# edogariu/artist-style-transfer

Hardware: NVIDIA B200
Metric: train_images_per_sec_256 (higher is better)
Workload: dtype bf16

## Files before the change

artist_style_transfer_b200/csrc/conv_px.cu:

```cuda
#include "px_common.cuh"

namespace ast {

constexpr int PX_THREADS = 320;
constexpr int PX_MAX_STAGES = 8;
constexpr int PX_PRODUCERS = 4;

struct PxParams {
  int mi, mj, tw, th, tiles_i, tiles_j, n_img;
  int ntaps, kchunks, kc;
  int si, so, oy0, ox0;
  int cout, flags;
  int w_rows_per_img;
  int stages, w_bytes, a_bytes, stage_bytes, rowb;
  int pairs_per_img;
  unsigned idesc, layout_type, sbo;
  long long total_pairs;
  short dy[AST_MAX_TAPS];
  short dx[AST_MAX_TAPS];
};

template <int KIND>
__global__ void __launch_bounds__(PX_THREADS, 1)
conv_px_kernel(const __grid_constant__ CUtensorMap tm_in, const __grid_constant__ CUtensorMap tm_w, const PxParams p,
               const float* __restrict__ bias, const Img32 add, const Img32 mask, const Img32 out,
               double* __restrict__ stats) {
  extern __shared__ unsigned char smem_raw[];
  __shared__ __align__(8) unsigned long long full_bar[PX_MAX_STAGES], empty_bar[PX_MAX_STAGES], tfull_bar[2], tempty_bar[2];
  __shared__ unsigned tmem_slot;
  unsigned char* smem = (unsigned char*)(((uintptr_t)smem_raw + 1023) & ~(uintptr_t)1023);
  const int warp = threadIdx.x >> 5, lane = threadIdx.x & 31;
  const int ksteps = p.ntaps * p.kchunks;

  if (threadIdx.x == 0) {
    asm volatile("prefetch.tensormap [%0];" ::"l"(&tm_in) : "memory");
    asm volatile("prefetch.tensormap [%0];" ::"l"(&tm_w) : "memory");
    for (int s = 0; s < p.stages; ++s) { mbar_init(&full_bar[s], 1); mbar_init(&empty_bar[s], 1); }
    for (int a = 0; a < 2; ++a) { mbar_init(&tfull_bar[a], 1); mbar_init(&tempty_bar[a], 256); }
    asm volatile("fence.mbarrier_init.release.cluster;" ::: "memory");
    asm volatile("fence.proxy.async.shared::cta;" ::: "memory");
  }
  if (warp == 1) {
    asm volatile("tcgen05.alloc.cta_group::1.sync.aligned.shared::cta.b32 [%0], %1;" ::"r"(smem_u32(&tmem_slot)), "r"(512u) : "memory");
    asm volatile("tcgen05.relinquish_alloc_permit.cta_group::1.sync.aligned;" ::: "memory");
  }
  tc_fence_before();
  __syncthreads();
  tc_fence_after();
  const unsigned tmem_base = tmem_slot;

  if (warp == 0) {
    const int nprod = p.stages < PX_PRODUCERS ? p.stages : PX_PRODUCERS;
    if (lane < nprod) {
      int s = 0, turn = 0; unsigned ph = 0;
      for (long long pair = blockIdx.x; pair < p.total_pairs; pair += gridDim.x) {
        const int img = (int)(pair / p.pairs_per_img);
        const int sp0 = 2 * (int)(pair % p.pairs_per_img);
        const int ti0 = sp0 / p.tiles_j, tj0 = sp0 - ti0 * p.tiles_j;
        const int ti1 = (sp0 + 1) / p.tiles_j, tj1 = (sp0 + 1) - ti1 * p.tiles_j;
        const int x0 = p.si * tj0 * p.tw, y0 = p.si * ti0 * p.th, x1 = p.si * tj1 * p.tw, y1 = p.si * ti1 * p.th;
        const int wrow0 = img * p.w_rows_per_img;
        for (int t = 0; t < p.ntaps; ++t) {
          for (int kc = 0; kc < p.kchunks; ++kc) {
            if (turn == lane) {
              mbar_wait(&empty_bar[s], ph ^ 1);
              unsigned char* sw = smem + (size_t)s * p.stage_bytes;
              mbar_expect_tx(&full_bar[s], (unsigned)p.stage_bytes);
              tma_load_2d(sw, &tm_w, &full_bar[s], kc * p.kc, wrow0 + t * p.cout);
              tma_load_4d(sw + p.w_bytes, &tm_in, &full_bar[s], kc * p.kc, x0 + p.dx[t], y0 + p.dy[t], img);
              tma_load_4d(sw + p.w_bytes + p.a_bytes, &tm_in, &full_bar[s], kc * p.kc, x1 + p.dx[t], y1 + p.dy[t], img);
            }
            if (++turn == nprod) turn = 0;
            if (++s == p.stages) { s = 0; ph ^= 1; }
          }
        }
      }
    }
  } else if (warp == 1) {
    int s = 0; unsigned ph = 0; int as = 0; unsigned aph = 0;
    const int kmma = p.rowb / 32;
    const unsigned desc_hi = (p.sbo >> 4) | (1u << 14) | (p.layout_type << 29);
    for (long long pair = blockIdx.x; pair < p.total_pairs; pair += gridDim.x) {
      mbar_wait(&tempty_bar[as], aph ^ 1);
      tc_fence_after();
      const unsigned d_tmem = tmem_base + (unsigned)(as * 256);
      for (int ks = 0; ks < ksteps; ++ks) {
        mbar_wait(&full_bar[s], ph);
        tc_fence_after();
        if (lane == 0) {
          const unsigned w_addr = smem_u32(smem + (size_t)s * p.stage_bytes);
          const unsigned a_lo = ((w_addr & 0x3FFFFu) >> 4) | (1u << 16);
          const unsigned b_lo = (((w_addr + p.w_bytes) & 0x3FFFFu) >> 4) | (1u << 16);
          tc_mma<KIND>(d_tmem, pack_desc64(a_lo, desc_hi), pack_desc64(b_lo, desc_hi), p.idesc, ks > 0 ? 1u : 0u);
          tc_mma<KIND>(d_tmem, pack_desc64(a_lo + 2, desc_hi), pack_desc64(b_lo + 2, desc_hi), p.idesc, 1u);
          if (kmma == 4) {
            tc_mma<KIND>(d_tmem, pack_desc64(a_lo + 4, desc_hi), pack_desc64(b_lo + 4, desc_hi), p.idesc, 1u);
            tc_mma<KIND>(d_tmem, pack_desc64(a_lo + 6, desc_hi), pack_desc64(b_lo + 6, desc_hi), p.idesc, 1u);
          }
          tc_commit(&empty_bar[s]);
          if (ks == ksteps - 1) tc_commit(&tfull_bar[as]);
        }
        __syncwarp();
        if (++s == p.stages) { s = 0; ph ^= 1; }
      }
      if (++as == 2) { as = 0; aph ^= 1; }
    }
  } else {
    const int q = warp & 3;
    const int half = (warp - 2) >> 2;
    const int ch = q * 32 + lane;
    const bool ch_ok = ch < p.cout;
    const float b = (bias && ch_ok) ? bias[ch] : 0.f;
    int as = 0; unsigned aph = 0;
    double s1 = 0.0, s2 = 0.0;
    int s_img = -1;
    for (long long pair = blockIdx.x; pair < p.total_pairs; pair += gridDim.x) {
      const int img = (int)(pair / p.pairs_per_img);
      if (stats && img != s_img) {
        if (s_img >= 0 && ch_ok) { double* srow = stats + ((long long)s_img * p.cout + ch) * 2; atomicAdd(srow, s1); atomicAdd(srow + 1, s2); }
        s1 = s2 = 0.0; s_img = img;
      }
      const int sp = 2 * (int)(pair % p.pairs_per_img) + half;
      const int ti = sp / p.tiles_j, tj = sp - ti * p.tiles_j;
      mbar_wait(&tfull_bar[as], aph);
      tc_fence_after();
      const unsigned taddr0 = tmem_base + ((unsigned)(q * 32) << 16) + (unsigned)(as * 256 + half * 128);
      if (q * 32 < p.cout) {
        const bool fast = (p.tw & 31) == 0;
        for (int c0 = 0; c0 < 128; c0 += 32) {
          float v[32];
          tc_ld32(taddr0 + c0, v);
          if (fast) {
            const int ty = c0 / p.tw, tx0 = c0 - ty * p.tw;
            const int i = ti * p.th + ty, j0 = tj * p.tw + tx0;
            const int oy = p.oy0 + p.so * i, ox = p.ox0 + p.so * j0;
            int nvalid = 0;
            if (i < p.mi && oy < out.h) {
              const int jlim = min(p.mj, (out.w - p.ox0 + p.so - 1) / p.so);
              nvalid = max(0, min(32, jlim - j0));
            }
            PxOff off;
            off.out = img * out.sn + oy * out.sh + ox * out.sw;
            off.add = add.ptr ? img * add.sn + oy * add.sh + ox * add.sw : 0;
            off.mask = mask.ptr ? img * mask.sn + oy * mask.sh + ox * mask.sw : 0;
            PxStep st;
            st.out_r = st.add_r = st.mask_r = 0;
            st.out_c = p.so * out.sw; st.add_c = p.so * add.sw; st.mask_c = p.so * mask.sw;
            if (nvalid > 0) px_chunk<32>(v, off, st, 1, nvalid, ch, lane, b, p.flags, add, mask, out, stats != nullptr, s1, s2);
          } else {
            const int row = c0 + lane;
            const int ty = row / p.tw, tx = row - ty * p.tw;
            const int i = ti * p.th + ty, j = tj * p.tw + tx;
            const int oy = p.oy0 + p.so * i, ox = p.ox0 + p.so * j;
            const bool valid = i < p.mi && j < p.mj && oy < out.h && ox < out.w;
            PxOff off;
            off.out = valid ? img * out.sn + oy * out.sh + ox * out.sw : -1;
            off.add = add.ptr ? img * add.sn + oy * add.sh + ox * add.sw : 0;
            off.mask = mask.ptr ? img * mask.sn + oy * mask.sh + ox * mask.sw : 0;
            PxStep st = {0, 0, 0, 0, 0, 0};
            px_chunk<0>(v, off, st, 0, 0, ch, lane, b, p.flags, add, mask, out, stats != nullptr, s1, s2);
          }
        }
      }
      tc_fence_before();
      mbar_arrive(&tempty_bar[as]);
      if (++as == 2) { as = 0; aph ^= 1; }
    }
    if (stats && s_img >= 0 && ch_ok) { double* srow = stats + ((long long)s_img * p.cout + ch) * 2; atomicAdd(srow, s1); atomicAdd(srow + 1, s2); }
  }

  tc_fence_before();
  __syncthreads();
  if (warp == 1) {
    tc_fence_after();
    asm volatile("tcgen05.dealloc.cta_group::1.sync.aligned.b32 %0, %1;" ::"r"(tmem_base), "r"(512u) : "memory");
  }
}

int conv_gather_px(const ast_image* in, const void* weights, const float* bias, const ast_image* add,
                   const ast_image* mask, const ast_image* out, const ast_gather_geom* g, int cpad, bool thin,
                   cudaStream_t stream) {
  if (thin || g->pooled || (cpad != 64 && cpad != 128) || out->c != cpad) return 0;
  if (!img32_ok(out) || !img32_ok(add) || !img32_ok(mask)) return 0;
  if (in->dtype == AST_F16) return 0;
  const int esz = in->dtype == AST_F32 ? 4 : 2;
  EncodeTiledFn encode = get_encode();
  if (!encode) return 0;

  PxParams p;
  memset(&p, 0, sizeof(p));
  p.mi = g->mi; p.mj = g->mj; p.si = g->si; p.so = g->so; p.oy0 = g->oy0; p.ox0 = g->ox0;
  p.ntaps = g->ntaps; p.flags = g->flags; p.cout = cpad; p.n_img = in->n;
  for (int t = 0; t < g->ntaps; ++t) { p.dy[t] = g->dy[t]; p.dx[t] = g->dx[t]; }
  pick_tile(p.mi, p.mj, 128, &p.tw, &p.th);
  p.tiles_i = (p.mi + p.th - 1) / p.th;
  p.tiles_j = (p.mj + p.tw - 1) / p.tw;
  p.rowb = (in->c * esz) % 128 == 0 ? 128 : 64;
  p.kc = p.rowb / esz;
  p.kchunks = in->c / p.kc;
  if (p.ntaps * p.kchunks * (p.rowb / 32) < 16) return 0;
  p.w_rows_per_img = 0;
  if (g->w_img_stride) {
    if (g->w_img_stride != (int64_t)g->ntaps * cpad * in->c) return 0;
    p.w_rows_per_img = g->ntaps * cpad;
  }
  p.w_bytes = 128 * p.rowb;
  p.a_bytes = 128 * p.rowb;
  p.stage_bytes = p.w_bytes + 2 * p.a_bytes;
  p.stages = (200 * 1024) / p.stage_bytes;
  if (p.stages > PX_MAX_STAGES) p.stages = PX_MAX_STAGES;
  p.layout_type = p.rowb == 128 ? 2u : 4u;
  p.sbo = 8u * p.rowb;
  const unsigned fmt = tc_operand_fmt(in->dtype);
  p.idesc = (1u << 4) | (fmt << 7) | (fmt << 10) | ((256u >> 3) << 17) | ((128u >> 4) << 24);
  p.pairs_per_img = (p.tiles_i * p.tiles_j + 1) / 2;
  p.total_pairs = (long long)p.n_img * p.pairs_per_img;

  alignas(64) CUtensorMap tm_in, tm_w;
  const CUtensorMapDataType dt = tc_tmap_dtype(in->dtype);
  const CUtensorMapSwizzle sw = p.rowb == 128 ? CU_TENSOR_MAP_SWIZZLE_128B : CU_TENSOR_MAP_SWIZZLE_64B;
  {
    cuuint64_t dims[4] = {(cuuint64_t)in->c, (cuuint64_t)in->w, (cuuint64_t)in->h, (cuuint64_t)in->n};
    cuuint64_t strides[3] = {(cuuint64_t)in->sw * esz, (cuuint64_t)in->sh * esz, (cuuint64_t)in->sn * esz};
    cuuint32_t box[4] = {(cuuint32_t)p.kc, (cuuint32_t)(p.tw * p.si), (cuuint32_t)(p.th * p.si), 1};
    cuuint32_t estr[4] = {1, (cuuint32_t)p.si, (cuuint32_t)p.si, 1};
    if (int r = cached_tensor_map(encode, &tm_in, dt, 4, in->ptr, dims, strides, box, estr, sw, CU_TENSOR_MAP_L2_PROMOTION_L2_128B)) return r;
  }
  {
    const long long rows = (long long)g->ntaps * cpad * (g->w_img_stride ? in->n : 1);
    cuuint64_t dims[2] = {(cuuint64_t)in->c, (cuuint64_t)rows};
    cuuint64_t strides[1] = {(cuuint64_t)in->c * esz};
    cuuint32_t box[2] = {(cuuint32_t)p.kc, 128};
    cuuint32_t estr[2] = {1, 1};
    if (int r = cached_tensor_map(encode, &tm_w, dt, 2, const_cast<void*>(weights), dims, strides, box, estr, sw, CU_TENSOR_MAP_L2_PROMOTION_L2_256B)) return r;
  }
  const size_t smem = (size_t)p.stages * p.stage_bytes + 1024;
  const int grid = (int)(p.total_pairs < num_sms() ? p.total_pairs : num_sms());
  cudaError_t e;
  if (in->dtype != AST_F32) {
    e = set_max_smem(conv_px_kernel<0>, smem);
    if (e == cudaSuccess) launch_k(conv_px_kernel<0>, grid, PX_THREADS, smem, stream, tm_in, tm_w, p, bias, to_img32(add), to_img32(mask), to_img32(out), g->stats);
  } else {
    e = set_max_smem(conv_px_kernel<1>, smem);
    if (e == cudaSuccess) launch_k(conv_px_kernel<1>, grid, PX_THREADS, smem, stream, tm_in, tm_w, p, bias, to_img32(add), to_img32(mask), to_img32(out), g->stats);
  }
  if (e != cudaSuccess) { set_error("conv_px: cudaFuncSetAttribute failed: %s", cudaGetErrorString(e)); return (int)e; }
  count_launch();
  count_work(FAM_CONV_PX, conv_flops(in, out, g), conv_bytes(in, out, g, add, mask));
  AST_CUDA_LAUNCH_CHECK();
  return 1;
}

}
```

Baseline: 3465.

## Use M=64 MMA for 64-channel convs, merge pair tiles into one TMA box

For 64-output-channel convolutions the kernel now issues MMAs with M equal to the padded channel count. It loads only cpad weight rows and reads TMEM with the 16x32bx2 layout, so it no longer wastes half the tensor-core work and weight bandwidth on padding. Producer lanes in one warp become separate producer warps (two extra warps, 384 threads). Vertically adjacent tile pairs are fetched with one doubled TMA box, the tile shape is chosen to minimise padding, and the epilogue takes a uniform full-chunk fast path. The per-channel cout guard is dropped and the warp/thread layout changes, which adds register pressure and correctness risk for the TMEM lane mapping.

```diff
diff --git a/artist_style_transfer_b200/csrc/conv_px.cu b/artist_style_transfer_b200/csrc/conv_px.cu
--- a/artist_style_transfer_b200/csrc/conv_px.cu
+++ b/artist_style_transfer_b200/csrc/conv_px.cu
@@ -2,9 +2,25 @@
 
 namespace ast {
 
-constexpr int PX_THREADS = 320;
+constexpr int PX_THREADS = 384;
 constexpr int PX_MAX_STAGES = 8;
-constexpr int PX_PRODUCERS = 4;
+constexpr int PX_PRODUCERS = 3;
+
+__device__ __forceinline__ void tc_ld16x2_32(unsigned taddr, float* v) {
+  unsigned r[32];
+  asm volatile(
+      "tcgen05.ld.sync.aligned.16x32bx2.x32.b32 "
+      "{%0, %1, %2, %3, %4, %5, %6, %7, %8, %9, %10, %11, %12, %13, %14, %15, "
+      "%16, %17, %18, %19, %20, %21, %22, %23, %24, %25, %26, %27, %28, %29, %30, %31}, [%32], 32;"
+      : "=r"(r[0]), "=r"(r[1]), "=r"(r[2]), "=r"(r[3]), "=r"(r[4]), "=r"(r[5]), "=r"(r[6]), "=r"(r[7]), "=r"(r[8]),
+        "=r"(r[9]), "=r"(r[10]), "=r"(r[11]), "=r"(r[12]), "=r"(r[13]), "=r"(r[14]), "=r"(r[15]), "=r"(r[16]),
+        "=r"(r[17]), "=r"(r[18]), "=r"(r[19]), "=r"(r[20]), "=r"(r[21]), "=r"(r[22]), "=r"(r[23]), "=r"(r[24]),
+        "=r"(r[25]), "=r"(r[26]), "=r"(r[27]), "=r"(r[28]), "=r"(r[29]), "=r"(r[30]), "=r"(r[31])
+      : "r"(taddr));
+  asm volatile("tcgen05.wait::ld.sync.aligned;" ::: "memory");
+#pragma unroll
+  for (int i = 0; i < 32; ++i) v[i] = __uint_as_float(r[i]);
+}
 
 struct PxParams {
   int mi, mj, tw, th, tiles_i, tiles_j, n_img;
@@ -13,6 +29,7 @@
   int cout, flags;
   int w_rows_per_img;
   int stages, w_bytes, a_bytes, stage_bytes, rowb;
+  int pair_box;
   int pairs_per_img;
   unsigned idesc, layout_type, sbo;
   long long total_pairs;
@@ -20,7 +37,7 @@
   short dx[AST_MAX_TAPS];
 };
 
-template <int KIND>
+template <int KIND, bool M64>
 __global__ void __launch_bounds__(PX_THREADS, 1)
 conv_px_kernel(const __grid_constant__ CUtensorMap tm_in, const __grid_constant__ CUtensorMap tm_w, const PxParams p,
                const float* __restrict__ bias, const Img32 add, const Img32 mask, const Img32 out,
@@ -49,9 +66,10 @@
   tc_fence_after();
   const unsigned tmem_base = tmem_slot;
 
-  if (warp == 0) {
+  if (warp == 0 || warp >= 10) {
     const int nprod = p.stages < PX_PRODUCERS ? p.stages : PX_PRODUCERS;
-    if (lane < nprod) {
+    const int pid = warp == 0 ? 0 : warp - 9;
+    if (lane == 0 && pid < nprod) {
       int s = 0, turn = 0; unsigned ph = 0;
       for (long long pair = blockIdx.x; pair < p.total_pairs; pair += gridDim.x) {
         const int img = (int)(pair / p.pairs_per_img);
@@ -62,13 +80,14 @@
         const int wrow0 = img * p.w_rows_per_img;
         for (int t = 0; t < p.ntaps; ++t) {
           for (int kc = 0; kc < p.kchunks; ++kc) {
-            if (turn == lane) {
+            if (turn == pid) {
               mbar_wait(&empty_bar[s], ph ^ 1);
               unsigned char* sw = smem + (size_t)s * p.stage_bytes;
               mbar_expect_tx(&full_bar[s], (unsigned)p.stage_bytes);
               tma_load_2d(sw, &tm_w, &full_bar[s], kc * p.kc, wrow0 + t * p.cout);
-              tma_load_4d(sw + p.w_bytes, &tm_in, &full_bar[s], kc * p.kc, x0 + p.dx[t], y0 + p.dy[t], img);
-              tma_load_4d(sw + p.w_bytes + p.a_bytes, &tm_in, &full_bar[s], kc * p.kc, x1 + p.dx[t], y1 + p.dy[t], img);
+              sw += p.w_bytes;
+              tma_load_4d(sw, &tm_in, &full_bar[s], kc * p.kc, x0 + p.dx[t], y0 + p.dy[t], img);
+              if (!p.pair_box) tma_load_4d(sw + p.a_bytes, &tm_in, &full_bar[s], kc * p.kc, x1 + p.dx[t], y1 + p.dy[t], img);
             }
             if (++turn == nprod) turn = 0;
             if (++s == p.stages) { s = 0; ph ^= 1; }
@@ -89,8 +108,9 @@
         tc_fence_after();
         if (lane == 0) {
           const unsigned w_addr = smem_u32(smem + (size_t)s * p.stage_bytes);
+          const unsigned x_addr = w_addr + p.w_bytes;
           const unsigned a_lo = ((w_addr & 0x3FFFFu) >> 4) | (1u << 16);
-          const unsigned b_lo = (((w_addr + p.w_bytes) & 0x3FFFFu) >> 4) | (1u << 16);
+          const unsigned b_lo = ((x_addr & 0x3FFFFu) >> 4) | (1u << 16);
           tc_mma<KIND>(d_tmem, pack_desc64(a_lo, desc_hi), pack_desc64(b_lo, desc_hi), p.idesc, ks > 0 ? 1u : 0u);
           tc_mma<KIND>(d_tmem, pack_desc64(a_lo + 2, desc_hi), pack_desc64(b_lo + 2, desc_hi), p.idesc, 1u);
           if (kmma == 4) {
@@ -108,16 +128,21 @@
   } else {
     const int q = warp & 3;
     const int half = (warp - 2) >> 2;
-    const int ch = q * 32 + lane;
-    const bool ch_ok = ch < p.cout;
-    const float b = (bias && ch_ok) ? bias[ch] : 0.f;
+    const int ch = M64 ? q * 16 + (lane & 15) : q * 32 + lane;
+    const int col_lane = M64 ? (lane >> 4) * 32 : 0;
+    constexpr int chunk = M64 ? 64 : 32;
+    const float b = bias ? bias[ch] : 0.f;
     int as = 0; unsigned aph = 0;
     double s1 = 0.0, s2 = 0.0;
     int s_img = -1;
+    auto flush = [&]() {
+      if (M64) { s1 += __shfl_xor_sync(0xffffffffu, s1, 16); s2 += __shfl_xor_sync(0xffffffffu, s2, 16); }
+      if (!M64 || lane < 16) { double* srow = stats + ((long long)s_img * p.cout + ch) * 2; atomicAdd(srow, s1); atomicAdd(srow + 1, s2); }
+    };
     for (long long pair = blockIdx.x; pair < p.total_pairs; pair += gridDim.x) {
       const int img = (int)(pair / p.pairs_per_img);
       if (stats && img != s_img) {
-        if (s_img >= 0 && ch_ok) { double* srow = stats + ((long long)s_img * p.cout + ch) * 2; atomicAdd(srow, s1); atomicAdd(srow + 1, s2); }
+        if (s_img >= 0) flush();
         s1 = s2 = 0.0; s_img = img;
       }
       const int sp = 2 * (int)(pair % p.pairs_per_img) + half;
@@ -125,48 +150,34 @@
       mbar_wait(&tfull_bar[as], aph);
       tc_fence_after();
       const unsigned taddr0 = tmem_base + ((unsigned)(q * 32) << 16) + (unsigned)(as * 256 + half * 128);
-      if (q * 32 < p.cout) {
-        const bool fast = (p.tw & 31) == 0;
-        for (int c0 = 0; c0 < 128; c0 += 32) {
-          float v[32];
-          tc_ld32(taddr0 + c0, v);
-          if (fast) {
-            const int ty = c0 / p.tw, tx0 = c0 - ty * p.tw;
-            const int i = ti * p.th + ty, j0 = tj * p.tw + tx0;
-            const int oy = p.oy0 + p.so * i, ox = p.ox0 + p.so * j0;
-            int nvalid = 0;
-            if (i < p.mi && oy < out.h) {
-              const int jlim = min(p.mj, (out.w - p.ox0 + p.so - 1) / p.so);
-              nvalid = max(0, min(32, jlim - j0));
-            }
-            PxOff off;
-            off.out = img * out.sn + oy * out.sh + ox * out.sw;
-            off.add = add.ptr ? img * add.sn + oy * add.sh + ox * add.sw : 0;
-            off.mask = mask.ptr ? img * mask.sn + oy * mask.sh + ox * mask.sw : 0;
-            PxStep st;
-            st.out_r = st.add_r = st.mask_r = 0;
-            st.out_c = p.so * out.sw; st.add_c = p.so * add.sw; st.mask_c = p.so * mask.sw;
-            if (nvalid > 0) px_chunk<32>(v, off, st, 1, nvalid, ch, lane, b, p.flags, add, mask, out, stats != nullptr, s1, s2);
-          } else {
-            const int row = c0 + lane;
-            const int ty = row / p.tw, tx = row - ty * p.tw;
-            const int i = ti * p.th + ty, j = tj * p.tw + tx;
-            const int oy = p.oy0 + p.so * i, ox = p.ox0 + p.so * j;
-            const bool valid = i < p.mi && j < p.mj && oy < out.h && ox < out.w;
-            PxOff off;
-            off.out = valid ? img * out.sn + oy * out.sh + ox * out.sw : -1;
-            off.add = add.ptr ? img * add.sn + oy * add.sh + ox * add.sw : 0;
-            off.mask = mask.ptr ? img * mask.sn + oy * mask.sh + ox * mask.sw : 0;
-            PxStep st = {0, 0, 0, 0, 0, 0};
-            px_chunk<0>(v, off, st, 0, 0, ch, lane, b, p.flags, add, mask, out, stats != nullptr, s1, s2);
-          }
-        }
+      for (int c0 = 0; c0 < 128; c0 += chunk) {
+        float v[32];
+        if (M64) tc_ld16x2_32(taddr0 + c0, v);
+        else tc_ld32(taddr0 + c0, v);
+        const int ilim = min(p.mi, (out.h - p.oy0 + p.so - 1) / p.so);
+        const int jlim = min(p.mj, (out.w - p.ox0 + p.so - 1) / p.so);
+        const int col = c0 + col_lane;
+        const int ty = col / p.tw, tx0 = col - ty * p.tw;
+        const int i = ti * p.th + ty, j0 = tj * p.tw + tx0;
+        const int nvalid = i < ilim ? max(0, min(32, jlim - j0)) : 0;
+        const int oy = p.oy0 + p.so * i, ox = p.ox0 + p.so * j0;
+        PxOff off;
+        off.out = img * out.sn + oy * out.sh + ox * out.sw;
+        off.add = add.ptr ? img * add.sn + oy * add.sh + ox * add.sw : 0;
+        off.mask = mask.ptr ? img * mask.sn + oy * mask.sh + ox * mask.sw : 0;
+        PxStep st;
+        st.out_r = p.so * out.sh; st.add_r = p.so * add.sh; st.mask_r = p.so * mask.sh;
+        st.out_c = p.so * out.sw; st.add_c = p.so * add.sw; st.mask_c = p.so * mask.sw;
+        if (__all_sync(0xffffffffu, nvalid == 32))
+          px_chunk<32, true>(v, off, st, 1, 32, ch, lane, b, p.flags, add, mask, out, stats != nullptr, s1, s2);
+        else if (__any_sync(0xffffffffu, nvalid > 0))
+          px_chunk<32>(v, off, st, 1, nvalid, ch, lane, b, p.flags, add, mask, out, stats != nullptr, s1, s2);
       }
       tc_fence_before();
       mbar_arrive(&tempty_bar[as]);
       if (++as == 2) { as = 0; aph ^= 1; }
     }
-    if (stats && s_img >= 0 && ch_ok) { double* srow = stats + ((long long)s_img * p.cout + ch) * 2; atomicAdd(srow, s1); atomicAdd(srow + 1, s2); }
+    if (stats && s_img >= 0) flush();
   }
 
   tc_fence_before();
@@ -175,6 +186,13 @@
     tc_fence_after();
     asm volatile("tcgen05.dealloc.cta_group::1.sync.aligned.b32 %0, %1;" ::"r"(tmem_base), "r"(512u) : "memory");
   }
+}
+
+typedef void (*PxLaunch)(const CUtensorMap, const CUtensorMap, const PxParams, const float*, const Img32, const Img32,
+                         const Img32, double*);
+static PxLaunch px_kernel(bool tf32, bool m64) {
+  if (tf32) return m64 ? conv_px_kernel<1, true> : conv_px_kernel<1, false>;
+  return m64 ? conv_px_kernel<0, true> : conv_px_kernel<0, false>;
 }
 
 int conv_gather_px(const ast_image* in, const void* weights, const float* bias, const ast_image* add,
@@ -192,7 +210,14 @@
   p.mi = g->mi; p.mj = g->mj; p.si = g->si; p.so = g->so; p.oy0 = g->oy0; p.ox0 = g->ox0;
   p.ntaps = g->ntaps; p.flags = g->flags; p.cout = cpad; p.n_img = in->n;
   for (int t = 0; t < g->ntaps; ++t) { p.dy[t] = g->dy[t]; p.dx[t] = g->dx[t]; }
-  pick_tile(p.mi, p.mj, 128, &p.tw, &p.th);
+  {
+    double best = -1;
+    for (int w = 128; w >= 32; w >>= 1) {
+      const int h = 128 / w;
+      const double eff = (double)p.mi * p.mj / ((double)((p.mi + h - 1) / h * h) * ((p.mj + w - 1) / w * w));
+      if (eff > best + 1e-9) { best = eff; p.tw = w; p.th = h; }
+    }
+  }
   p.tiles_i = (p.mi + p.th - 1) / p.th;
   p.tiles_j = (p.mj + p.tw - 1) / p.tw;
   p.rowb = (in->c * esz) % 128 == 0 ? 128 : 64;
@@ -204,7 +229,7 @@
     if (g->w_img_stride != (int64_t)g->ntaps * cpad * in->c) return 0;
     p.w_rows_per_img = g->ntaps * cpad;
   }
-  p.w_bytes = 128 * p.rowb;
+  p.w_bytes = cpad * p.rowb;
   p.a_bytes = 128 * p.rowb;
   p.stage_bytes = p.w_bytes + 2 * p.a_bytes;
   p.stages = (200 * 1024) / p.stage_bytes;
@@ -212,8 +237,9 @@
   p.layout_type = p.rowb == 128 ? 2u : 4u;
   p.sbo = 8u * p.rowb;
   const unsigned fmt = tc_operand_fmt(in->dtype);
-  p.idesc = (1u << 4) | (fmt << 7) | (fmt << 10) | ((256u >> 3) << 17) | ((128u >> 4) << 24);
+  p.idesc = (1u << 4) | (fmt << 7) | (fmt << 10) | ((256u >> 3) << 17) | (((unsigned)cpad >> 4) << 24);
   p.pairs_per_img = (p.tiles_i * p.tiles_j + 1) / 2;
+  p.pair_box = p.tiles_j == 1 && 2 * p.th * p.si <= 256;
   p.total_pairs = (long long)p.n_img * p.pairs_per_img;
 
   alignas(64) CUtensorMap tm_in, tm_w;
@@ -222,7 +248,7 @@
   {
     cuuint64_t dims[4] = {(cuuint64_t)in->c, (cuuint64_t)in->w, (cuuint64_t)in->h, (cuuint64_t)in->n};
     cuuint64_t strides[3] = {(cuuint64_t)in->sw * esz, (cuuint64_t)in->sh * esz, (cuuint64_t)in->sn * esz};
-    cuuint32_t box[4] = {(cuuint32_t)p.kc, (cuuint32_t)(p.tw * p.si), (cuuint32_t)(p.th * p.si), 1};
+    cuuint32_t box[4] = {(cuuint32_t)p.kc, (cuuint32_t)(p.tw * p.si), (cuuint32_t)((p.pair_box ? 2 : 1) * p.th * p.si), 1};
     cuuint32_t estr[4] = {1, (cuuint32_t)p.si, (cuuint32_t)p.si, 1};
     if (int r = cached_tensor_map(encode, &tm_in, dt, 4, in->ptr, dims, strides, box, estr, sw, CU_TENSOR_MAP_L2_PROMOTION_L2_128B)) return r;
   }
@@ -230,20 +256,15 @@
     const long long rows = (long long)g->ntaps * cpad * (g->w_img_stride ? in->n : 1);
     cuuint64_t dims[2] = {(cuuint64_t)in->c, (cuuint64_t)rows};
     cuuint64_t strides[1] = {(cuuint64_t)in->c * esz};
-    cuuint32_t box[2] = {(cuuint32_t)p.kc, 128};
+    cuuint32_t box[2] = {(cuuint32_t)p.kc, (cuuint32_t)cpad};
     cuuint32_t estr[2] = {1, 1};
     if (int r = cached_tensor_map(encode, &tm_w, dt, 2, const_cast<void*>(weights), dims, strides, box, estr, sw, CU_TENSOR_MAP_L2_PROMOTION_L2_256B)) return r;
   }
   const size_t smem = (size_t)p.stages * p.stage_bytes + 1024;
   const int grid = (int)(p.total_pairs < num_sms() ? p.total_pairs : num_sms());
-  cudaError_t e;
-  if (in->dtype != AST_F32) {
-    e = set_max_smem(conv_px_kernel<0>, smem);
-    if (e == cudaSuccess) launch_k(conv_px_kernel<0>, grid, PX_THREADS, smem, stream, tm_in, tm_w, p, bias, to_img32(add), to_img32(mask), to_img32(out), g->stats);
-  } else {
-    e = set_max_smem(conv_px_kernel<1>, smem);
-    if (e == cudaSuccess) launch_k(conv_px_kernel<1>, grid, PX_THREADS, smem, stream, tm_in, tm_w, p, bias, to_img32(add), to_img32(mask), to_img32(out), g->stats);
-  }
+  const PxLaunch launch = px_kernel(in->dtype == AST_F32, cpad == 64);
+  cudaError_t e = set_max_smem(launch, smem);
+  if (e == cudaSuccess) launch_k(launch, grid, PX_THREADS, smem, stream, tm_in, tm_w, p, bias, to_img32(add), to_img32(mask), to_img32(out), g->stats);
   if (e != cudaSuccess) { set_error("conv_px: cudaFuncSetAttribute failed: %s", cudaGetErrorString(e)); return (int)e; }
   count_launch();
   count_work(FAM_CONV_PX, conv_flops(in, out, g), conv_bytes(in, out, g, add, mask));
diff --git a/scratch/conv_px_launches.py b/scratch/conv_px_launches.py
--- /dev/null
+++ b/scratch/conv_px_launches.py
@@ -0,0 +1,98 @@
+import argparse
+import json
+import os
+import subprocess
+import sys
+
+ROOT = os.path.dirname(os.path.dirname(os.path.abspath(__file__)))
+sys.path.insert(0, ROOT)
+
+import torch
+
+import artist_style_transfer_b200 as ast
+from artist_style_transfer_b200 import _lib, ops
+
+MMA_TFS = 1380.0
+HBM_GBS = 6500.0
+
+
+def device_info():
+    q = subprocess.run(["nvidia-smi", "--query-gpu=name,power.limit,clocks.max.sm", "--format=csv,noheader"],
+                       capture_output=True, text=True).stdout.strip().splitlines()
+    return f"{torch.cuda.get_device_name()} | nvidia-smi: {q[torch.cuda.current_device()] if q else 'n/a'}"
+
+
+def main():
+    ap = argparse.ArgumentParser()
+    ap.add_argument("--tag", default="")
+    ap.add_argument("--iters", type=int, default=50)
+    ap.add_argument("--reps", type=int, default=5)
+    ap.add_argument("--json", default="")
+    a = ap.parse_args()
+    assert torch.cuda.is_available(), "needs a GPU"
+    dev = torch.device("cuda:0")
+    torch.manual_seed(0)
+    net = ast.StyleTransfer(device=dev, precision="fast")
+    vgg = ast.VGG16(vgg_path=None, precision="fast").to(dev)
+    g = torch.Generator(device=dev).manual_seed(5)
+    content = torch.randint(0, 256, (32, 3, 256, 256), device=dev, generator=g).float()
+    style = ast.style_grams_single(vgg, torch.randint(0, 256, (3, 256, 256), device=dev, generator=g).float(), 32)
+
+    calls = []
+    orig = ops.conv_gather
+
+    def wrapped(x, wpacked, launches, out, **kw):
+        before = _lib.family_stats()["conv_px"][0]
+        r = orig(x, wpacked, launches, out, **kw)
+        if _lib.family_stats()["conv_px"][0] != before:
+            torch.cuda.synchronize()
+            keep = {k: (v.clone() if torch.is_tensor(v) else v) for k, v in kw.items()}
+            calls.append((x.clone(), wpacked.clone(), launches, out.clone(), keep))
+        return r
+
+    ops.conv_gather = wrapped
+    ast.perceptual_step(net, vgg, content, style)
+    torch.cuda.synchronize()
+    ops.conv_gather = orig
+    print(device_info(), a.tag, flush=True)
+    rows = []
+    for x, wp, launches, out, kw in calls:
+        xs = [x, x.clone()]
+        outs = [out, out.clone()]
+        def go(i):
+            ops.conv_gather(xs[i & 1], wp, launches, outs[i & 1], **kw)
+        for i in range(4):
+            go(i)
+        torch.cuda.synchronize()
+        ts = []
+        for _ in range(a.reps):
+            e0, e1 = torch.cuda.Event(enable_timing=True), torch.cuda.Event(enable_timing=True)
+            e0.record()
+            for i in range(a.iters):
+                go(i)
+            e1.record()
+            torch.cuda.synchronize()
+            ts.append(e0.elapsed_time(e1) / a.iters * 1e3)
+        us = sorted(ts)[len(ts) // 2]
+        n, cin, cout = x.shape[0], x.shape[-1], out.shape[-1]
+        flop = 2.0 * n * sum(l.mi * l.mj * len(l.taps) for l in launches) * cin * cout
+        byts = x.numel() * x.element_size() + out.numel() * out.element_size()
+        for k in ("add", "mask"):
+            if kw.get(k) is not None:
+                byts += kw[k].numel() * kw[k].element_size()
+        epi = ",".join(k for k in ("bias", "add", "mask", "stats") if kw.get(k) is not None) + (",relu" if kw.get("relu") else "")
+        row = dict(x=list(x.shape), out=list(out.shape), dtype=str(x.dtype)[6:], taps=sum(len(l.taps) for l in launches),
+                   epi=epi or "-", us=round(us, 1), spread=round(max(ts) - min(ts), 1), tfs=round(flop / us / 1e6, 1),
+                   gflop=round(flop / 1e9, 2), mb=round(byts / 1e6, 1), mma_floor_us=round(flop / MMA_TFS / 1e6, 1),
+                   hbm_floor_us=round(byts / HBM_GBS / 1e3, 1))
+        rows.append(row)
+        print(json.dumps(row), flush=True)
+    print(f"total {sum(r['us'] for r in rows):.1f} us over {len(rows)} launches", flush=True)
+    if a.json:
+        os.makedirs(os.path.dirname(a.json) or ".", exist_ok=True)
+        with open(a.json, "w") as f:
+            json.dump(dict(device=device_info(), tag=a.tag, rows=rows), f, indent=1)
+
+
+if __name__ == "__main__":
+    main()
```

New measurement: 3517, median of 6. +1.5%, better.
